# ZhangHH233/Retinal_OCT_Image_Segmentation_via_Deep_Learning

Measured on NVIDIA B200. Metric: bscans_per_sec_full_metric_suite, higher is better.
Workload: dtype u8

## Files before the change

retinal_oct_image_segmentation_via_deep_learning_b200/csrc/contour.cu:

```cuda
#include <cstdlib>
#include <cstring>
#include <numeric>
#include <type_traits>

#include <mutex>

#include "common.cuh"
#include "trace_core.h"

namespace octm {

struct TraceParams {
    const uint8_t* yt;
    const uint8_t* yp;
    long long n_items;
    int H, W, K, max_pts;
    const uint32_t* first_pos;
    uint32_t* verts;
    uint32_t* n_pts;
    uint32_t* flags;
    const int* bnd_t;
    const int* bnd_p;
    bool only_todo;
    const uint32_t* todo_count;
// ... 1133 lines not shown
                else break;
            }
            digit = static_cast<uint32_t>(lane * 8 + d);
            knew = k - run;
        }
        const int src = __ffs(__ballot_sync(0xffffffffu, mine)) - 1;
        digit = __shfl_sync(0xffffffffu, digit, src);
        k = __shfl_sync(0xffffffffu, knew, src);
        prefix |= digit << shift;
        maskbits |= 255u << shift;
        __syncwarp();
    }
    return prefix;
}

__global__ void __launch_bounds__(128) distance_select_kernel(const SelectParams prm) {
    __shared__ uint32_t s_hist[4][256];
    const int lane = threadIdx.x & 31, warp = threadIdx.x >> 5;
    const int cap = prm.max_pts;
    if (prm.todo_count != nullptr && *prm.todo_count == 0) return;
    for (long long unit = static_cast<long long>(blockIdx.x) * 4 + warp; unit < prm.n_units;
         unit += static_cast<long long>(gridDim.x) * 4) {
        const long long pair = unit >> 1;
        const int dir = static_cast<int>(unit & 1);
        if (prm.max_sq[unit] != kNeedsSelect) continue;
        const int nq = static_cast<int>(min(prm.n_pts[pair * 2 + 1 - dir], static_cast<uint32_t>(cap)));
        const uint32_t* dq = prm.d2 + unit * static_cast<long long>(cap);
        uint32_t vmax = 0;
        double dsum = 0.0;
        {
            double ds[4] = {0.0, 0.0, 0.0, 0.0};
            int j = lane;
            for (; j + 96 < nq; j += 128) {
                uint32_t v[4];
#pragma unroll
                for (int u = 0; u < 4; ++u) v[u] = dq[j + 32 * u];
#pragma unroll
                for (int u = 0; u < 4; ++u) {
                    vmax = max(vmax, v[u]);
                    ds[u] += sqrt(static_cast<double>(v[u]) / 4.0);
                }
            }
            double dt = 0.0;
            for (; j < nq; j += 32) {
                const uint32_t v = dq[j];
                vmax = max(vmax, v);
                dt += sqrt(static_cast<double>(v) / 4.0);
            }
            dsum = ((ds[0] + ds[1]) + (ds[2] + ds[3])) + dt;
        }
        vmax = __reduce_max_sync(0xffffffffu, vmax);
#pragma unroll
        for (int o = 16; o > 0; o >>= 1) dsum += __shfl_xor_sync(0xffffffffu, dsum, o);
        const double pos = __dmul_rn(static_cast<double>(nq - 1), 0.95);
        const uint32_t lo = static_cast<uint32_t>(floor(pos));
        const uint32_t v_lo = warp_select(dq, nq, lo, vmax, s_hist[warp], lane);
        uint32_t cnt_le = 0, next_gt = 0xffffffffu;
#pragma unroll 4
        for (int j = lane; j < nq; j += 32) {
            const uint32_t v = dq[j];
            cnt_le += v <= v_lo ? 1u : 0u;
            if (v > v_lo) next_gt = min(next_gt, v);
        }
        cnt_le = __reduce_add_sync(0xffffffffu, cnt_le);
        next_gt = __reduce_min_sync(0xffffffffu, next_gt);
        const uint32_t v_hi = (lo + 1 >= static_cast<uint32_t>(nq) || cnt_le >= lo + 2) ? v_lo : next_gt;
        if (lane == 0) {
            prm.max_sq[unit] = vmax;
            prm.p95_sq[unit * 2 + 0] = v_lo;
            prm.p95_sq[unit * 2 + 1] = v_hi;
            prm.sum_dist[unit] = dsum;
        }
    }
}


constexpr int kLdWarps = 4;
constexpr int kLdPad = 32;
constexpr int kLdRing = 512;
constexpr int kLdShort = 64;
#ifndef OCTM_LD_MINB
#define OCTM_LD_MINB 8
#endif

struct LayeredDistParams {
    const uint32_t* first_pos;
    const int* bnd_t;
    const int* bnd_p;
    const uint32_t* unsorted;
    long long n_pairs;
    int H, W, K, max_pts;
    int tab;
    uint32_t* verts;
    uint32_t* n_pts;
    uint32_t* max_sq;
    uint32_t* p95_sq;
    double* sum_dist;
    uint32_t* todo_count;
    uint32_t* search_count;
    int vals_cap;
};

__device__ __forceinline__ int max3i(int a, int b, int c) { return max(max(a, b), c); }
__device__ __forceinline__ int min3i(int a, int b, int c) { return min(min(a, b), c); }

__device__ __forceinline__ void layered_nearest2p(const short* lo0, const short* hi0, const short* lo1, const short* hi1, int qy0,
                                                  int qx0, int qy1, int qx1, int ncol, int& best0, int& best1) {
    const short* l0 = lo0 + qx0;
    const short* h0 = hi0 + qx0;
    const short* l1 = lo1 + qx1;
    const short* h1 = hi1 + qx1;
    const int dy0 = max3i(l0[0] - qy0, qy0 - h0[0], 0), dy1 = max3i(l1[0] - qy1, qy1 - h1[0], 0);
    best0 = dy0 * dy0;
    best1 = dy1 * dy1;
    int d = 1;
    while (d * d < max(best0, best1) && d < kLdPad) {
        const int d2 = d * d, e2 = (d + 1) * (d + 1);
        {
            const int a0 = max3i(l0[-d] - qy0, qy0 - h0[-d], 1), a1 = max3i(l0[d] - qy0, qy0 - h0[d], 1);
            const int b0 = max3i(l0[-d - 1] - qy0, qy0 - h0[-d - 1], 0), b1 = max3i(l0[d + 1] - qy0, qy0 - h0[d + 1], 0);
            best0 = min3i(best0, a0 * a0 + d2, a1 * a1 + d2);
            best0 = min3i(best0, b0 * b0 + e2, b1 * b1 + e2);
        }
        {
            const int a0 = max3i(l1[-d] - qy1, qy1 - h1[-d], 1), a1 = max3i(l1[d] - qy1, qy1 - h1[d], 1);
            const int b0 = max3i(l1[-d - 1] - qy1, qy1 - h1[-d - 1], 0), b1 = max3i(l1[d + 1] - qy1, qy1 - h1[d + 1], 0);
            best1 = min3i(best1, a0 * a0 + d2, a1 * a1 + d2);
            best1 = min3i(best1, b0 * b0 + e2, b1 * b1 + e2);
        }
        d += 2;
    }
    for (int e = d; e * e < best0; ++e) {
        const int cl = max(qx0 - e, -1), cr = min(qx0 + e, ncol), par = e & 1;
        const int a0 = max3i(lo0[cl] - qy0, qy0 - hi0[cl], par), a1 = max3i(lo0[cr] - qy0, qy0 - hi0[cr], par);
        best0 = min3i(best0, a0 * a0 + e * e, a1 * a1 + e * e);
    }
    for (int e = d; e * e < best1; ++e) {
        const int cl = max(qx1 - e, -1), cr = min(qx1 + e, ncol), par = e & 1;
        const int a0 = max3i(lo1[cl] - qy1, qy1 - hi1[cl], par), a1 = max3i(lo1[cr] - qy1, qy1 - hi1[cr], par);
        best1 = min3i(best1, a0 * a0 + e * e, a1 * a1 + e * e);
    }
}
__device__ __forceinline__ void layered_nearest2(const short* lo, const short* hi, int qy0, int qx0, int qy1, int qx1,
                                                 int ncol, int& best0, int& best1) {
    layered_nearest2p(lo, hi, lo, hi, qy0, qx0, qy1, qx1, ncol, best0, best1);
}

__device__ __forceinline__ void list_nearest2(const int2* pts, int n, int qy0, int qx0, int qy1, int qx1, int& best0, int& best1) {
    best0 = best1 = 0x7fffffff;
#pragma unroll 2
    for (int i = 0; i < n; ++i) {
        const int2 v = pts[i];
        const int dy0 = v.x - qy0, dx0 = v.y - qx0, dy1 = v.x - qy1, dx1 = v.y - qx1;
        best0 = min(best0, dy0 * dy0 + dx0 * dx0);
        best1 = min(best1, dy1 * dy1 + dx1 * dx1);
    }
}

struct LdSide {
    const short* lo;
    const short* hi;
    const int2* pts;
    const int* best;
    int n;
};

template <bool SRC_TABLE>
__device__ __forceinline__ void ld_list_minima(const int2* qpts, int nq, const LdSide& src, int ncol, int tid, int* best) {
    for (int q = 0; q < nq; ++q) {
        const int2 v = qpts[q];
        int b = 0x7fffffff;
        if (SRC_TABLE) {
            for (int c = tid; c < ncol; c += kLdWarps * 32) {
                const int dx = c - v.y;
                const int dy = max3i(src.lo[c] - v.x, v.x - src.hi[c], dx & 1);
                b = min(b, dy * dy + dx * dx);
            }
        } else {
            for (int i = tid; i < src.n; i += kLdWarps * 32) {
                const int dy = src.pts[i].x - v.x, dx = src.pts[i].y - v.y;
                b = min(b, dy * dy + dx * dx);
            }
        }
        b = __reduce_min_sync(0xffffffffu, b);
        if ((tid & 31) == 0) atomicMin(&best[q], b);
    }
}

template <bool SRC_TABLE>
__device__ __forceinline__ void ld_nearest2(const LdSide& src, int qy0, int qx0, int qy1, int qx1, int ncol, int& b0, int& b1) {
    if (SRC_TABLE) layered_nearest2(src.lo, src.hi, qy0, qx0, qy1, qx1, ncol, b0, b1);
    else list_nearest2(src.pts, src.n, qy0, qx0, qy1, qx1, b0, b1);
}

struct FineCounter {
    uint32_t* bins;
    uint32_t run_max = 0;
    bool run_bad = false, overflow = false;
    __device__ __forceinline__ void add(int best, bool valid, int lane) { count_minima(best, valid, lane, bins, run_max, run_bad); }
};
struct WideCounter {
    uint32_t* bins;
    int mode;
    int shift;
    uint32_t target;
    uint32_t run_max = 0, next_min = 0xffffffffu;
    double sum = 0.0;
    bool run_bad = false, overflow = false;
    uint32_t* vals = nullptr;
    uint32_t* vals_n = nullptr;
    __device__ __forceinline__ void add(int best, bool valid, int lane) {
        if (mode == 0) {
            count_minima(best, valid, lane, bins, run_max, run_bad);
            return;
        }
        if (mode == 1 && vals != nullptr) {
            const uint32_t m = __ballot_sync(0xffffffffu, valid);
            uint32_t base = 0;
            if (lane == 0 && m) base = atomicAdd(vals_n, static_cast<uint32_t>(__popc(m)));
            base = __shfl_sync(0xffffffffu, base, 0);
            if (valid) vals[base + __popc(m & lanemask_lt())] = static_cast<uint32_t>(best);
        }
        const uint32_t v = static_cast<uint32_t>(best), key = v >> shift;
        if (valid) run_max = max(run_max, v);
        const bool in = valid && (mode == 1 || key == target);
        const uint32_t idx = mode == 1 ? key : (v & ((1u << shift) - 1u)) >> 1;
        const uint32_t peers = __match_any_sync(0xffffffffu, in ? idx : static_cast<uint32_t>(kCountBins) + lane);
        if (in && lane == __ffs(peers) - 1) atomicAdd(&bins[idx >> 1], static_cast<uint32_t>(__popc(peers)) << ((idx & 1u) * 16));
// ... 69 lines not shown
        ld_nearest2<SRC_TABLE>(src, static_cast<int>(q0 >> 16), static_cast<int>(q0 & 0xffffu), static_cast<int>(q1 >> 16),
                               static_cast<int>(q1 & 0xffffu), ncol, b0, b1);
        ctr.add(b0, v0, lane);
        ctr.add(b1, v1, lane);
    }
}

__device__ __forceinline__ void ld_list_stats(const int* best, int n, int lane, uint32_t* max_sq, uint32_t* p95_sq, double* sum_dist) {
    const bool v0 = lane < n, v1 = lane + 32 < n;
    const uint32_t a = v0 ? static_cast<uint32_t>(best[lane]) : 0u, b = v1 ? static_cast<uint32_t>(best[lane + 32]) : 0u;
    uint32_t ra = 0, rb = 0;
    for (int i = 0; i < n; ++i) {
        const uint32_t w = static_cast<uint32_t>(best[i]);
        ra += (w < a || (w == a && i < lane)) ? 1u : 0u;
        rb += (w < b || (w == b && i < lane + 32)) ? 1u : 0u;
    }
    const double pos = __dmul_rn(static_cast<double>(n - 1), 0.95);
    const uint32_t lo = static_cast<uint32_t>(floor(pos)), hi = lo + 1 < static_cast<uint32_t>(n) ? lo + 1 : lo;
    uint32_t v_lo = 0, v_hi = 0;
    uint32_t m = __ballot_sync(0xffffffffu, v0 && ra == lo);
    if (m) v_lo = __shfl_sync(0xffffffffu, a, __ffs(m) - 1);
    m = __ballot_sync(0xffffffffu, v1 && rb == lo);
    if (m) v_lo = __shfl_sync(0xffffffffu, b, __ffs(m) - 1);
    m = __ballot_sync(0xffffffffu, v0 && ra == hi);
    if (m) v_hi = __shfl_sync(0xffffffffu, a, __ffs(m) - 1);
    m = __ballot_sync(0xffffffffu, v1 && rb == hi);
    if (m) v_hi = __shfl_sync(0xffffffffu, b, __ffs(m) - 1);
    const uint32_t vmax = __reduce_max_sync(0xffffffffu, max(a, b));
    double ds = __dadd_rn(v0 ? sqrt(static_cast<double>(a) / 4.0) : 0.0, v1 ? sqrt(static_cast<double>(b) / 4.0) : 0.0);
#pragma unroll
    for (int o = 16; o > 0; o >>= 1) ds = __dadd_rn(ds, __shfl_xor_sync(0xffffffffu, ds, o));
    if (lane == 0) {
        *max_sq = vmax;
        p95_sq[0] = v_lo;
        p95_sq[1] = v_hi;
        *sum_dist = ds;
    }
}

__device__ __forceinline__ void ld_table_vs_list(const short* qlo, const short* qhi, const int2* pts, int n, int W, int nq, int tid,
                                                 uint32_t* vals, uint32_t* s_nvals, uint32_t* s_scr , double* s_dscr ,
                                                 uint32_t* s_hist , uint32_t* s_bc , uint32_t* max_sq, uint32_t* p95_sq,
                                                 double* sum_dist) {
    uint32_t vmax = 0;
    double dsum = 0.0;
    auto emit = [&](int qy, int qx) {
        int best = 0x7fffffff;
        for (int i = 0; i < n; ++i) {
            const int2 v = pts[i];
            const int dy = v.x - qy, dx = v.y - qx;
            best = min(best, dy * dy + dx * dx);
        }
        vals[atomicAdd(s_nvals, 1u)] = static_cast<uint32_t>(best);
        vmax = max(vmax, static_cast<uint32_t>(best));
        dsum = __dadd_rn(dsum, sqrt(static_cast<double>(best) / 4.0));
    };
    for (int x = tid; x < W; x += kLdWarps * 32) {
        emit(qlo[2 * x], 2 * x);
        if (x + 1 < W)
            for (int y = qlo[2 * x + 1], yh = qhi[2 * x + 1]; y <= yh; y += 2) emit(y, 2 * x + 1);
    }
    vmax = block_reduce_max<kLdWarps * 32>(vmax, s_scr);
    dsum = block_reduce_add<kLdWarps * 32>(dsum, s_dscr);
    const double pos = __dmul_rn(static_cast<double>(nq - 1), 0.95);
    const uint32_t lo = static_cast<uint32_t>(floor(pos));
    const uint32_t v_lo = block_select<kLdWarps * 32>(vals, nq, lo, vmax, s_hist, s_bc);
    uint32_t cnt_le = 0, next_gt = 0xffffffffu;
    for (int j = tid; j < nq; j += kLdWarps * 32) {
        const uint32_t v = vals[j];
        cnt_le += v <= v_lo ? 1u : 0u;
        if (v > v_lo) next_gt = min(next_gt, v);
    }
    cnt_le = block_reduce_add<kLdWarps * 32>(cnt_le, s_scr);
    next_gt = block_reduce_min<kLdWarps * 32>(next_gt, s_scr);
    const uint32_t v_hi = (lo + 1 >= static_cast<uint32_t>(nq) || cnt_le >= lo + 2) ? v_lo : next_gt;
    if (tid == 0) {
        *max_sq = vmax;
        p95_sq[0] = v_lo;
        p95_sq[1] = v_hi;
        *sum_dist = dsum;
    }
}

__device__ __forceinline__ void ld_both_tt(const short* tabs, int tab, int W, int ncol, int warp, int lane, uint32_t* ring,
                                           uint32_t* bins2, uint32_t* s_vmax, uint32_t* s_bad) {
    uint32_t rm0 = 0, rm1 = 0, head = 0, tail = 0;
    bool bad0 = false, bad1 = false, overflow = false;
    const int nblk = (W + 63) >> 6;
    auto count = [&](int bestd, bool valid, uint32_t dirq) {
        const uint32_t dv = static_cast<uint32_t>(bestd), h = dv >> 1;
        const bool ok = valid && (dv & 1u) == 0 && h < static_cast<uint32_t>(kCountBins);
        const uint32_t peers = __match_any_sync(0xffffffffu, ok ? (h | (dirq << 16)) : 0x100000u + lane);
        if (ok && lane == __ffs(peers) - 1)
            atomicAdd(&bins2[dirq * (kCountBins / 2) + (h >> 1)], static_cast<uint32_t>(__popc(peers)) << ((h & 1u) * 16));
        if (valid) {
            if (dirq) rm1 = max(rm1, dv); else rm0 = max(rm0, dv);
            if (!ok) { if (dirq) bad1 = true; else bad0 = true; }
        }
    };
    auto ring_round = [&](uint32_t left) {
        const bool v0 = static_cast<uint32_t>(lane) < left, v1 = static_cast<uint32_t>(lane) + 32u < left;
        const uint32_t idle = static_cast<uint32_t>(static_cast<unsigned short>(tabs[kLdPad])) << 16;
        const uint32_t q0 = v0 ? ring[(head + lane) & (kLdRing - 1)] : idle, q1 = v1 ? ring[(head + 32 + lane) & (kLdRing - 1)] : idle;
        head += left < 64u ? left : 64u;
        const uint32_t d0 = q0 >> 31, d1 = q1 >> 31;
        const short* lo0 = tabs + kLdPad + d0 * (2 * tab);
        const short* lo1 = tabs + kLdPad + d1 * (2 * tab);
        int b0, b1;
        layered_nearest2p(lo0, lo0 + tab, lo1, lo1 + tab, static_cast<int>((q0 >> 16) & 0x7fffu), static_cast<int>(q0 & 0xffffu),
                          static_cast<int>((q1 >> 16) & 0x7fffu), static_cast<int>(q1 & 0xffffu), ncol, b0, b1);
        count(b0, v0, d0);
        count(b1, v1, d1);
    };
#pragma unroll 1
    for (int dir = 0; dir < 2 && !overflow; ++dir) {
        const short* slo = tabs + kLdPad + dir * (2 * tab);
        const short* shi = slo + tab;
        const short* qlo = tabs + kLdPad + (1 - dir) * (2 * tab);
        const short* qhi = qlo + tab;
        const uint32_t tag = static_cast<uint32_t>(dir) << 31;
        const int idle_y = slo[0];
        for (int blk = warp; blk < nblk; blk += kLdWarps) {
            const int xa = blk * 64 + lane, xb = xa + 32;
            const bool va = xa < W, vb = xb < W;
            int ba, bb;
            layered_nearest2(slo, shi, va ? qlo[2 * xa] : idle_y, va ? 2 * xa : 0, vb ? qlo[2 * xb] : idle_y, vb ? 2 * xb : 0, ncol, ba, bb);
            count(ba, va, static_cast<uint32_t>(dir));
            count(bb, vb, static_cast<uint32_t>(dir));
            const bool ra = xa + 1 < W, rb = xb + 1 < W;
            const int la = ra ? qlo[2 * xa + 1] : 32767, ha = ra ? qhi[2 * xa + 1] : -32768;
            const int lb = rb ? qlo[2 * xb + 1] : 32767, hb = rb ? qhi[2 * xb + 1] : -32768;
            const uint32_t lena = ha >= la ? static_cast<uint32_t>((ha - la) >> 1) + 1u : 0u;
            const uint32_t lenb = hb >= lb ? static_cast<uint32_t>((hb - lb) >> 1) + 1u : 0u;
            const uint32_t len = lena + lenb;
            uint32_t incl = len;
#pragma unroll
            for (int o = 1; o < 32; o <<= 1) {
                const uint32_t up = __shfl_up_sync(0xffffffffu, incl, o);
                if (lane >= o) incl += up;
            }
            const uint32_t total = __shfl_sync(0xffffffffu, incl, 31);
            if (total > static_cast<uint32_t>(kLdRing - 64)) { overflow = true; break; }
            uint32_t at = tail + incl - len;
            for (uint32_t t = 0; t < lena; ++t, ++at)
                ring[at & (kLdRing - 1)] = tag | (static_cast<uint32_t>(la + 2 * static_cast<int>(t)) << 16) | static_cast<uint32_t>(2 * xa + 1);
            for (uint32_t t = 0; t < lenb; ++t, ++at)
                ring[at & (kLdRing - 1)] = tag | (static_cast<uint32_t>(lb + 2 * static_cast<int>(t)) << 16) | static_cast<uint32_t>(2 * xb + 1);
            tail += total;
            __syncwarp();
            while (tail - head >= 64u) ring_round(64u);
            __syncwarp();
        }
    }
    if (!overflow && tail != head) ring_round(tail - head);
    const uint32_t w0 = __reduce_max_sync(0xffffffffu, rm0), w1 = __reduce_max_sync(0xffffffffu, rm1);
    const bool b0 = __any_sync(0xffffffffu, bad0), b1 = __any_sync(0xffffffffu, bad1), ov = __any_sync(0xffffffffu, overflow);
    if (lane == 0) {
        atomicMax(&s_vmax[0], w0);
        atomicMax(&s_vmax[1], w1);
        if (b0 || b1 || ov) atomicOr(s_bad, (b0 ? 1u : 0u) | (b1 ? 2u : 0u) | (ov ? 4u : 0u));
    }
}

__device__ __forceinline__ void ld_emit(const short* lo, const short* hi, int ncol, int lane, uint32_t* out, uint32_t cap) {
    uint32_t base = 0;
    for (int c0 = 0; c0 < ncol; c0 += 32) {
        const int c = c0 + lane;
        const int l = c < ncol ? lo[c] : 32767, h = c < ncol ? hi[c] : -32768;
        const uint32_t len = h >= l ? static_cast<uint32_t>((h - l) >> 1) + 1u : 0u;
        uint32_t incl = len;
#pragma unroll
        for (int o = 1; o < 32; o <<= 1) {
            const uint32_t up = __shfl_up_sync(0xffffffffu, incl, o);
            if (lane >= o) incl += up;
        }
        uint32_t at = base + incl - len;
        for (uint32_t t = 0; t < len; ++t, ++at)
            if (at < cap) out[at] = (static_cast<uint32_t>(l + 2 * static_cast<int>(t)) << 16) | static_cast<uint32_t>(c);
        base += __shfl_sync(0xffffffffu, incl, 31);
    }
}

template <int PASS>
__global__ void __launch_bounds__(kLdWarps * 32, PASS != 2 ? OCTM_LD_MINB : 8) layered_distance_kernel(const LayeredDistParams prm) {
    extern __shared__ __align__(16) uint8_t dsm[];
    __shared__ uint32_t s_vmax[2], s_bad, s_ok[2], s_minkey[2], s_cnt[2], s_seed[2];
    __shared__ int2 s_list[2][kLdShort];
    __shared__ int s_lbest[2][kLdShort];
    __shared__ double s_dsum[kLdWarps];
    __shared__ double s_dsum8[8];
    __shared__ uint32_t s_next, s_tgt[3], s_amax, s_nvals;
    constexpr bool P1 = PASS == 1 || PASS == 3;
    const int tid = threadIdx.x, lane = tid & 31, warp = tid >> 5;
    const int W = prm.W, K = prm.K, tab = prm.tab, ncol = 2 * W - 1;
    if (PASS == 2 && *prm.todo_count == 0) return;
    short* const tabs = reinterpret_cast<short*>(dsm);
    uint32_t* const bins2 = reinterpret_cast<uint32_t*>(dsm + static_cast<size_t>(tab) * 8);
    uint32_t* const ring = bins2 + kCountBins + warp * kLdRing;
    for (int i = tid; i < kCountBins; i += kLdWarps * 32) bins2[i] = 0;
    for (int i = tid; i < 2 * tab; i += kLdWarps * 32) {
        const int m = i >= tab ? 1 : 0, j = i - m * tab;
        if (j < kLdPad || j >= kLdPad + ncol) {
            tabs[(2 * m) * tab + j] = 32767;
            tabs[(2 * m + 1) * tab + j] = -32768;
        }
    }

    for (long long pair0 = blockIdx.x; pair0 < prm.n_pairs; pair0 += gridDim.x) {
      bool own_next = false;
      for (int rep = 0; rep < 2; ++rep) {
        if (rep == 1 && !own_next) break;
        const long long pair = pair0 + rep;
        if (PASS == 2 && prm.max_sq[pair * 2] != kNeedsSearch) continue;
        __syncthreads();
        const long long item = pair / K;
        const int cls = static_cast<int>(pair - item * K);
        if (P1 && rep == 0) {
            const uint32_t ft = lane < K ? prm.first_pos[(item * 2 + 0) * K + lane] : OCTM_NO_SEED;
            const uint32_t fq = lane < K ? prm.first_pos[(item * 2 + 1) * K + lane] : OCTM_NO_SEED;
            const int c00t = __ffs(__ballot_sync(0xffffffffu, ft == 0u)) - 1, c00p = __ffs(__ballot_sync(0xffffffffu, fq == 0u)) - 1;
            if (c00t >= 0 && c00t == c00p && (PASS != 3 || (prm.unsorted[item] & 3u) == 0u)) {
                if (cls == c00t + 1) break;
                own_next = cls == c00t && cls + 1 < K;
            }
        }
        if (tid < 2) { s_vmax[tid] = 0; s_ok[tid] = 1; s_minkey[tid] = 0xffffffffu; s_cnt[tid] = 0; }
        if (tid == 2) s_bad = 0;
        const uint32_t unsorted = P1 ? prm.unsorted[item] : 0u;
        uint32_t n0 = 0, n1 = 0;
        if (PASS == 2 || (PASS == 3 && (unsorted & 1u))) n0 = prm.n_pts[pair * 2];
        if (PASS == 2 || (PASS == 3 && (unsorted & 2u))) n1 = prm.n_pts[pair * 2 + 1];
        const bool row0 = PASS == 3 && (unsorted & 1u) && n0 != kTraceTodo && (n0 & kRowBit);
        const bool row1 = PASS == 3 && (unsorted & 2u) && n1 != kTraceTodo && (n1 & kRowBit);
        __syncthreads();
        {
            const int m = warp >> 1;
            const uint32_t nm = m ? n1 : n0;
            const bool rowside = PASS == 3 && ((unsorted >> m) & 1u) && nm != kTraceTodo && (nm & kRowBit);
            const bool want = P1 || (nm != kTraceTodo && (nm & kLayeredBit));
            const uint32_t* fp = prm.first_pos + (item * 2 + m) * K;
            const uint32_t myfp = lane < K ? fp[lane] : OCTM_NO_SEED;
            const int c00 = __ffs(__ballot_sync(0xffffffffu, myfp == 0u)) - 1;
            const bool inv = cls == c00;
            const uint32_t others = __reduce_min_sync(0xffffffffu, lane == c00 ? OCTM_NO_SEED : myfp);
            const uint32_t seed = inv ? others : __shfl_sync(0xffffffffu, myfp, cls);
            if (lane == 0 && (warp & 1) == 0) s_seed[m] = seed;
            const int brow = inv ? cls : cls - 1;
            if (want && seed != OCTM_NO_SEED && (!((unsorted >> m) & 1u) || rowside) && brow >= 0 && brow < K - 1) {
                const int* rows = (m ? prm.bnd_p : prm.bnd_t) + item * (K - 1) * static_cast<long long>(W);
                const int* hrow = rows + brow * static_cast<long long>(W);
                if ((PASS == 2 && (nm & kRowBit)) || rowside)
                    hrow = reinterpret_cast<const int*>(prm.verts + (pair * 2 + m) * static_cast<long long>(prm.max_pts));
                const int* orow = inv ? (cls > 0 ? rows + (cls - 1) * static_cast<long long>(W) : nullptr)
                                      : (cls < K - 1 ? rows + cls * static_cast<long long>(W) : nullptr);
                if (PASS == 2 || rowside) orow = nullptr;
                uint32_t* lo32 = reinterpret_cast<uint32_t*>(tabs + (2 * m) * tab + kLdPad);
                uint32_t* hi32 = lo32 + (tab >> 1);
                bool ok = true;
                uint32_t minkey = 0xffffffffu, steps = 0;
                const int H = prm.H;
                const bool vec4 = (W & 3) == 0 && ((reinterpret_cast<uintptr_t>(hrow) | reinterpret_cast<uintptr_t>(orow)) & 15) == 0;
                for (int x0 = (warp & 1) * 128; vec4 && x0 < W; x0 += 256) {
                    const int x = x0 + 4 * lane;
                    const int xc = min(x, W - 4);
                    const int4 hv = *reinterpret_cast<const int4*>(hrow + xc);
                    const int4 ov = orow != nullptr ? *reinterpret_cast<const int4*>(orow + xc) : (inv ? make_int4(0, 0, 0, 0) : make_int4(H, H, H, H));
                    int hl = __shfl_up_sync(0xffffffffu, hv.w, 1), hn = __shfl_down_sync(0xffffffffu, hv.x, 1);
                    if (lane == 0) hl = hrow[max(xc - 1, 0)];
                    if (lane == 31) hn = hrow[min(xc + 4, W - 1)];
                    if (x + 4 >= W) hn = hv.w;
                    if (x < W) {
                        const int hh[6] = {hl, hv.x, hv.y, hv.z, hv.w, hn};
                        const int oo[4] = {ov.x, ov.y, ov.z, ov.w};
                        uint32_t wl[4], wh[4];
#pragma unroll
                        for (int i = 0; i < 4; ++i) {
                            const int h = hh[i + 1], hp = hh[i], hx = hh[i + 2];
                            if (P1) {
                                const int lo_w = min(hp, min(h, hx)), hi_w = max(hp, max(h, hx));
                                ok = ok && h >= 1 && h <= H - 1 && (inv ? oo[i] <= lo_w - 1 : oo[i] >= hi_w + 1);
                                minkey = min(minkey, static_cast<uint32_t>(h) * static_cast<uint32_t>(W) + static_cast<uint32_t>(x + i));
// ... 517 lines not shown
        if (smem > static_cast<size_t>(octm::max_optin_smem()))
            return octm::fail(OCTM_ERR_UNSUPPORTED, "tile %d needs %zu B of shared memory", tile, smem);
        if (cudaFuncSetAttribute(octm::distance_search_kernel, cudaFuncAttributeMaxDynamicSharedMemorySize,
                                 static_cast<int>(smem)) != cudaSuccess)
            return octm::fail(OCTM_ERR_LAUNCH, "cudaFuncSetAttribute(distance_search_kernel) failed");
        octm::SearchParams sp{verts, n_pts, n_pairs * 2, max_pts, tile, d2, max_sq, p95_sq, sum_dist, keep_d2 != 0, only_marked, todo_count};
        long long grid = n_pairs * 2;
        const long long cap = static_cast<long long>(octm::sm_count()) * 32;
        if (grid > cap) grid = cap;
        OCTM_TIMED("distance_search_kernel", st) octm::distance_search_kernel<<<static_cast<unsigned>(grid), octm::kSearchThreads, smem, st>>>(sp);
        if (int e = octm::check_launch("distance_search_kernel")) return e;
        return run_select();
    }
    const size_t smem = dist_smem(max_pts);
    if (smem > static_cast<size_t>(octm::max_optin_smem()) - 4096)
        return octm::fail(OCTM_ERR_UNSUPPORTED, "max_pts %d needs %zu B of shared memory in this mode", max_pts, smem);
    octm::DistParams p{verts, n_pts, n_pairs, max_pts, max_sq, p95_sq, sum_dist, d2};
    long long grid = n_pairs;
    const long long cap = static_cast<long long>(octm::sm_count()) * 16;
    if (grid > cap) grid = cap;
    auto kern = mode == 2 ? octm::distance_kernel<false> : octm::distance_kernel<true>;
    if (cudaFuncSetAttribute(kern, cudaFuncAttributeMaxDynamicSharedMemorySize, octm::max_optin_smem() - 4096) != cudaSuccess)
        return octm::fail(OCTM_ERR_LAUNCH, "cudaFuncSetAttribute(distance_kernel) failed");
    OCTM_TIMED("distance_kernel", st) kern<<<static_cast<unsigned>(grid), octm::kDistThreads, smem, st>>>(p);
    return octm::check_launch("distance_kernel");
}

extern "C" int octm_contour2d_distance(const uint32_t* verts, const uint32_t* n_pts, int64_t n_items, int num_classes,
                                       int max_pts, int H, int W, uint32_t* max_sq, uint32_t* p95_sq, double* sum_dist,
                                       uint32_t* d2, int keep_d2, void* stream) {
    return run_distance(verts, n_pts, n_items, num_classes, max_pts, H, W, max_sq, p95_sq, sum_dist, d2, keep_d2, false, nullptr, stream);
}

namespace octm {
__global__ void walk_report_kernel(const uint32_t* walk_count, uint32_t contours, uint32_t* out) {
    out[1] = contours;
    out[0] = *walk_count;
}
struct WalkReport {
    uint32_t* host = nullptr;
    uint32_t* dev = nullptr;
};
static WalkReport g_walk_report[64];
static std::mutex g_walk_mu;
static WalkReport* walk_report() {
    int dev = -1;
    if (cudaGetDevice(&dev) != cudaSuccess || dev < 0 || dev >= 64) { cudaGetLastError(); return nullptr; }
    std::lock_guard<std::mutex> lk(g_walk_mu);
    WalkReport& r = g_walk_report[dev];
    if (r.host == nullptr) {
        void* h = nullptr;
        void* d = nullptr;
        if (cudaHostAlloc(&h, 2 * sizeof(uint32_t), cudaHostAllocMapped) != cudaSuccess || cudaHostGetDevicePointer(&d, h, 0) != cudaSuccess) {
            cudaGetLastError();
            return nullptr;
        }
        r.host = static_cast<uint32_t*>(h);
        r.dev = static_cast<uint32_t*>(d);
        r.host[0] = r.host[1] = 0;
    }
    return &r;
}
}

extern "C" int octm_contour2d_metrics_u8(const uint8_t* y_true, const uint8_t* y_pred, int64_t n_items, int H, int W,
                                         int num_classes, const uint32_t* first_pos, const int32_t* bnd_true,
                                         const int32_t* bnd_pred, const uint32_t* unsorted, int max_pts, uint32_t* n_pts,
                                         uint32_t* flags, uint32_t* max_sq, uint32_t* p95_sq, double* sum_dist,
                                         void* workspace, size_t workspace_bytes, void* stream) {
    if (int e = check_shape(n_items, H, W, num_classes, max_pts)) return e;
    if (n_items == 0) return OCTM_OK;
    if (!y_true || !y_pred || !first_pos || !n_pts || !flags || !max_sq || !p95_sq || !sum_dist)
        return octm::fail(OCTM_ERR_INVALID, "null pointer");
    if ((bnd_true == nullptr) != (bnd_pred == nullptr)) return octm::fail(OCTM_ERR_INVALID, "bnd_true/bnd_pred: both or neither");
    const size_t verts_b = (static_cast<size_t>(n_items) * num_classes * 2 * max_pts * sizeof(uint32_t) + 255) & ~static_cast<size_t>(255);
    if (workspace == nullptr || workspace_bytes < 2 * verts_b + 256)
        return octm::fail(OCTM_ERR_WORKSPACE, "workspace too small: need %zu B", 2 * verts_b + 256);
    uint32_t* verts = static_cast<uint32_t*>(workspace);
    uint32_t* d2 = reinterpret_cast<uint32_t*>(static_cast<uint8_t*>(workspace) + verts_b);
    uint32_t* todo = reinterpret_cast<uint32_t*>(static_cast<uint8_t*>(workspace) + 2 * verts_b);
    cudaStream_t s = static_cast<cudaStream_t>(stream);
    static const bool env_fused = [] { const char* e = getenv("OCTM_LAYERED_FUSED"); return !(e && e[0] == '0'); }();
    const int tab = (2 * W - 1 + 2 * octm::kLdPad + 7) & ~7;
    const size_t smem = static_cast<size_t>(tab) * 8 + octm::kCountBins * 4 + octm::kLdWarps * octm::kLdRing * 4;
    const bool fused = env_fused && unsorted != nullptr && layered_ok(y_true, y_pred, bnd_true, bnd_pred, H, W, num_classes) &&
                       H <= 4095 && max_pts <= 0xffff && smem <= static_cast<size_t>(octm::max_optin_smem());
    if (!fused) {
        if (int e = octm_contour2d_trace_u8(y_true, y_pred, n_items, H, W, num_classes, first_pos, bnd_true, bnd_pred, max_pts,
                                            verts, n_pts, flags, stream))
            return e;
        return run_distance(verts, n_pts, n_items, num_classes, max_pts, H, W, max_sq, p95_sq, sum_dist, d2, 0, false, nullptr, stream);
    }
    if (cudaMemsetAsync(flags, 0, sizeof(uint32_t) * n_items * num_classes, s) != cudaSuccess ||
        cudaMemsetAsync(todo, 0, 3 * sizeof(uint32_t), s) != cudaSuccess)
        return octm::fail(OCTM_ERR_LAUNCH, "memset(flags) failed");
    uint32_t* search = todo + 1;
    const long long n_pairs = n_items * num_classes;
    octm::LayeredDistParams lp{first_pos, bnd_true, bnd_pred, unsorted, n_pairs, H, W, num_classes, max_pts, tab, verts,
                               n_pts, max_sq, p95_sq, sum_dist, todo, search, 0};
    auto launch_fused = [&](int pass) -> int {
        auto kern = pass == 1 ? octm::layered_distance_kernel<1> : (pass == 3 ? octm::layered_distance_kernel<3> : octm::layered_distance_kernel<2>);
        size_t smem_pass = smem;
        lp.vals_cap = 0;
        if (pass == 2 && max_pts <= 4096) {
            smem_pass += static_cast<size_t>(max_pts) * 4;
            lp.vals_cap = max_pts;
        }
        const size_t smem = smem_pass;
        if (cudaFuncSetAttribute(kern, cudaFuncAttributeMaxDynamicSharedMemorySize, static_cast<int>(smem)) != cudaSuccess)
            return octm::fail(OCTM_ERR_LAUNCH, "cudaFuncSetAttribute(layered_distance_kernel) failed");
        int fit = 0;
        if (cudaOccupancyMaxActiveBlocksPerMultiprocessor(&fit, kern, octm::kLdWarps * 32, smem) != cudaSuccess || fit < 1) {
            cudaGetLastError();
            fit = 1;
        }
        static const int env_ctas = [] { const char* e = getenv("OCTM_LD_CTAS"); return e ? atoi(e) : 0; }();
        if (env_ctas > 0 && env_ctas < fit) fit = env_ctas;
        long long grid = n_pairs;
        const long long cap = static_cast<long long>(octm::sm_count()) * fit;
        if (grid > cap) grid = cap;
        while (grid > 1 && std::gcd(grid, static_cast<long long>(num_classes)) != 1) --grid;
        OCTM_TIMED(pass == 1 ? "layered_distance_kernel" : (pass == 3 ? "layered_distance_kernel_rows" : "layered_distance_kernel_pass2"), s)
            kern<<<static_cast<unsigned>(grid), octm::kLdWarps * 32, smem, s>>>(lp);
        return octm::check_launch("layered_distance_kernel");
    };
    octm::TraceParams p{y_true, y_pred, n_items, H, W, num_classes, max_pts, first_pos, verts, n_pts, flags,
                        bnd_true, bnd_pred, true, todo, d2, todo + 2, 0, unsorted, 0};
    octm::WalkReport* wr = octm::stream_mostly_rejected() ? octm::walk_report() : nullptr;
    const bool few_walks = wr != nullptr && (octm_label_pass_seed_policy(-1) == 2 ||
                                             static_cast<unsigned long long>(*static_cast<volatile uint32_t*>(wr->host)) * 4ull <=
                                                 *static_cast<volatile uint32_t*>(wr->host + 1));
    if (wr != nullptr && few_walks) {
        p.take = 1;
        p.todo_count = nullptr;
        if (int e = launch_layered_trace<false>(p, s)) return e;
        p.todo_count = todo;
        if (int e = launch_fused(3)) return e;
        p.take = 2;
    } else {
        if (int e = launch_fused(1)) return e;
    }
    if (int e = launch_layered_trace<false>(p, s)) return e;
    p.take = 0;
    if (wr != nullptr) {
        OCTM_TIMED("walk_report_kernel", s) octm::walk_report_kernel<<<1, 1, 0, s>>>(
            todo + 2, static_cast<uint32_t>(std::min<long long>(n_items * num_classes * 2, 0xffffffffll)), wr->dev);
        if (int e = octm::check_launch("walk_report_kernel")) return e;
    }
    if (int e = launch_walk(p, s)) return e;
    if (int e = launch_fused(2)) return e;
    return run_distance(verts, n_pts, n_items, num_classes, max_pts, H, W, max_sq, p95_sq, sum_dist, d2, 0, true, search, stream);
}

extern "C" size_t octm_contour2d_workspace_bytes(int64_t n_items, int H, int W, int num_classes, int max_pts) {
    (void)H; (void)W;
    if (n_items <= 0 || num_classes < 1 || max_pts < 1) return 0;
    const size_t verts = static_cast<size_t>(n_items) * num_classes * 2 * max_pts * sizeof(uint32_t);
    const size_t first = static_cast<size_t>(n_items) * 2 * num_classes * sizeof(uint32_t);
    return 2 * ((verts + 255) & ~static_cast<size_t>(255)) + ((first + 255) & ~static_cast<size_t>(255));
}

extern "C" int octm_contour2d_u8(const uint8_t* y_true, const uint8_t* y_pred, int64_t n_items, int H, int W,
                                 int num_classes, const uint32_t* first_pos, int max_pts, uint32_t* n_pts,
                                 uint32_t* flags, uint32_t* max_sq, uint32_t* p95_sq, double* sum_dist, void* workspace,
                                 size_t workspace_bytes, void* stream) {
    if (int e = check_shape(n_items, H, W, num_classes, max_pts)) return e;
    if (n_items == 0) return OCTM_OK;
    if (workspace == nullptr || workspace_bytes < octm_contour2d_workspace_bytes(n_items, H, W, num_classes, max_pts))
        return octm::fail(OCTM_ERR_WORKSPACE, "workspace too small: need %zu B",
                          octm_contour2d_workspace_bytes(n_items, H, W, num_classes, max_pts));
    uint32_t* verts = static_cast<uint32_t*>(workspace);
    const size_t verts_b = (static_cast<size_t>(n_items) * num_classes * 2 * max_pts * sizeof(uint32_t) + 255) & ~static_cast<size_t>(255);
    uint32_t* d2_ws = reinterpret_cast<uint32_t*>(static_cast<uint8_t*>(workspace) + verts_b);
    uint32_t* fp_ws = reinterpret_cast<uint32_t*>(static_cast<uint8_t*>(workspace) + 2 * verts_b);
    if (first_pos == nullptr) {
        const long long grid = n_items < 148 * 8 ? n_items : 148 * 8;
        cudaStream_t s = static_cast<cudaStream_t>(stream);
        OCTM_TIMED("first_pos_kernel", s) octm::first_pos_kernel<<<static_cast<unsigned>(grid), 256, 0, s>>>(y_true, n_items, static_cast<long long>(H) * W,
                                                                         num_classes, fp_ws, 2 * num_classes);
        if (int e = octm::check_launch("first_pos_kernel")) return e;
        OCTM_TIMED("first_pos_kernel", s) octm::first_pos_kernel<<<static_cast<unsigned>(grid), 256, 0, s>>>(y_pred, n_items, static_cast<long long>(H) * W,
                                                                         num_classes, fp_ws + num_classes, 2 * num_classes);
        if (int e = octm::check_launch("first_pos_kernel")) return e;
        first_pos = fp_ws;
    }
// ... 6 lines not shown
```

Before: 3.407 million.

## Restructure layered nearest search into per-lane slot scheduler with work queue

```diff
diff --git a/retinal_oct_image_segmentation_via_deep_learning_b200/csrc/contour.cu b/retinal_oct_image_segmentation_via_deep_learning_b200/csrc/contour.cu
--- a/retinal_oct_image_segmentation_via_deep_learning_b200/csrc/contour.cu
+++ b/retinal_oct_image_segmentation_via_deep_learning_b200/csrc/contour.cu
@@ -1239,6 +1239,14 @@
 #ifndef OCTM_LD_MINB
 #define OCTM_LD_MINB 8
 #endif
+#ifndef OCTM_LD_SLOTS
+#define OCTM_LD_SLOTS 2
+#endif
+constexpr int kLdSlots = OCTM_LD_SLOTS;
+constexpr int kLdQueue = 128;
+constexpr int kLdCbuf = 128;
+static_assert(32 * (kLdSlots + 1) <= kLdQueue && 32 * (kLdSlots + 1) <= kLdCbuf, "PASS 1 queue sizes");
+__host__ __device__ constexpr int ld_warp_words(int pass) { return pass == 2 ? kLdRing : kLdQueue + kLdCbuf; }
 
 struct LayeredDistParams {
     const uint32_t* first_pos;
@@ -1261,12 +1269,21 @@
 __device__ __forceinline__ int max3i(int a, int b, int c) { return max(max(a, b), c); }
 __device__ __forceinline__ int min3i(int a, int b, int c) { return min(min(a, b), c); }
 
-__device__ __forceinline__ void layered_nearest2p(const short* lo0, const short* hi0, const short* lo1, const short* hi1, int qy0,
-                                                  int qx0, int qy1, int qx1, int ncol, int& best0, int& best1) {
-    const short* l0 = lo0 + qx0;
-    const short* h0 = hi0 + qx0;
-    const short* l1 = lo1 + qx1;
-    const short* h1 = hi1 + qx1;
+__device__ __forceinline__ int layered_far(const short* lo, const short* hi, int qy, int qx, int ncol, int d, int best) {
+    for (int e = d; e * e < best; ++e) {
+        const int cl = max(qx - e, -1), cr = min(qx + e, ncol), par = e & 1;
+        const int a0 = max3i(lo[cl] - qy, qy - hi[cl], par), a1 = max3i(lo[cr] - qy, qy - hi[cr], par);
+        best = min3i(best, a0 * a0 + e * e, a1 * a1 + e * e);
+    }
+    return best;
+}
+
+__device__ __forceinline__ void layered_nearest2(const short* lo, const short* hi, int qy0, int qx0, int qy1, int qx1,
+                                                 int ncol, int& best0, int& best1) {
+    const short* l0 = lo + qx0;
+    const short* h0 = hi + qx0;
+    const short* l1 = lo + qx1;
+    const short* h1 = hi + qx1;
     const int dy0 = max3i(l0[0] - qy0, qy0 - h0[0], 0), dy1 = max3i(l1[0] - qy1, qy1 - h1[0], 0);
     best0 = dy0 * dy0;
     best1 = dy1 * dy1;
@@ -1287,20 +1304,8 @@
         }
         d += 2;
     }
-    for (int e = d; e * e < best0; ++e) {
-        const int cl = max(qx0 - e, -1), cr = min(qx0 + e, ncol), par = e & 1;
-        const int a0 = max3i(lo0[cl] - qy0, qy0 - hi0[cl], par), a1 = max3i(lo0[cr] - qy0, qy0 - hi0[cr], par);
-        best0 = min3i(best0, a0 * a0 + e * e, a1 * a1 + e * e);
-    }
-    for (int e = d; e * e < best1; ++e) {
-        const int cl = max(qx1 - e, -1), cr = min(qx1 + e, ncol), par = e & 1;
-        const int a0 = max3i(lo1[cl] - qy1, qy1 - hi1[cl], par), a1 = max3i(lo1[cr] - qy1, qy1 - hi1[cr], par);
-        best1 = min3i(best1, a0 * a0 + e * e, a1 * a1 + e * e);
-    }
-}
-__device__ __forceinline__ void layered_nearest2(const short* lo, const short* hi, int qy0, int qx0, int qy1, int qx1,
-                                                 int ncol, int& best0, int& best1) {
-    layered_nearest2p(lo, hi, lo, hi, qy0, qx0, qy1, qx1, ncol, best0, best1);
+    best0 = layered_far(lo, hi, qy0, qx0, ncol, d, best0);
+    best1 = layered_far(lo, hi, qy1, qx1, ncol, d, best1);
 }
 
 __device__ __forceinline__ void list_nearest2(const int2* pts, int n, int qy0, int qx0, int qy1, int qx1, int& best0, int& best1) {
@@ -1536,15 +1541,16 @@
     }
 }
 
-__device__ __forceinline__ void ld_both_tt(const short* tabs, int tab, int W, int ncol, int warp, int lane, uint32_t* ring,
+__device__ __forceinline__ void ld_both_tt(const short* tabs, int tab, int W, int ncol, int warp, int lane, uint32_t* queue,
                                            uint32_t* bins2, uint32_t* s_vmax, uint32_t* s_bad) {
-    uint32_t rm0 = 0, rm1 = 0, head = 0, tail = 0;
+    constexpr uint32_t kAll = 0xffffffffu, kNoSeg = 0x80000000u;
+    uint32_t* const cbuf = queue + kLdQueue;
+    uint32_t rm0 = 0, rm1 = 0;
     bool bad0 = false, bad1 = false, overflow = false;
-    const int nblk = (W + 63) >> 6;
-    auto count = [&](int bestd, bool valid, uint32_t dirq) {
-        const uint32_t dv = static_cast<uint32_t>(bestd), h = dv >> 1;
+    auto count = [&](uint32_t v, bool valid) {
+        const uint32_t dirq = v >> 31, dv = v & 0x7fffffffu, h = dv >> 1;
         const bool ok = valid && (dv & 1u) == 0 && h < static_cast<uint32_t>(kCountBins);
-        const uint32_t peers = __match_any_sync(0xffffffffu, ok ? (h | (dirq << 16)) : 0x100000u + lane);
+        const uint32_t peers = __match_any_sync(kAll, ok ? (h | (dirq << 16)) : 0x100000u + lane);
         if (ok && lane == __ffs(peers) - 1)
             atomicAdd(&bins2[dirq * (kCountBins / 2) + (h >> 1)], static_cast<uint32_t>(__popc(peers)) << ((h & 1u) * 16));
         if (valid) {
@@ -1552,63 +1558,140 @@
             if (!ok) { if (dirq) bad1 = true; else bad0 = true; }
         }
     };
-    auto ring_round = [&](uint32_t left) {
-        const bool v0 = static_cast<uint32_t>(lane) < left, v1 = static_cast<uint32_t>(lane) + 32u < left;
-        const uint32_t idle = static_cast<uint32_t>(static_cast<unsigned short>(tabs[kLdPad])) << 16;
-        const uint32_t q0 = v0 ? ring[(head + lane) & (kLdRing - 1)] : idle, q1 = v1 ? ring[(head + 32 + lane) & (kLdRing - 1)] : idle;
-        head += left < 64u ? left : 64u;
-        const uint32_t d0 = q0 >> 31, d1 = q1 >> 31;
-        const short* lo0 = tabs + kLdPad + d0 * (2 * tab);
-        const short* lo1 = tabs + kLdPad + d1 * (2 * tab);
-        int b0, b1;
-        layered_nearest2p(lo0, lo0 + tab, lo1, lo1 + tab, static_cast<int>((q0 >> 16) & 0x7fffu), static_cast<int>(q0 & 0xffffu),
-                          static_cast<int>((q1 >> 16) & 0x7fffu), static_cast<int>(q1 & 0xffffu), ncol, b0, b1);
-        count(b0, v0, d0);
-        count(b1, v1, d1);
+    const int nblk = (W + 63) >> 6;
+    int g = warp, x0 = 0, qoff = 0, cseg = -1;
+    uint32_t tag = 0, total = 0, pos = 0, cstart = 0, sa = kNoSeg, sb = kNoSeg;
+    uint32_t qhead = 0, qtail = 0, chead = 0, ctail = 0;
+    auto load_block = [&]() {
+        const int dir = g >= nblk ? 1 : 0;
+        x0 = (g - dir * nblk) * 64;
+        qoff = kLdPad + (1 - dir) * (2 * tab);
+        tag = static_cast<uint32_t>(dir) << 31;
+        auto seg_len = [&](int x) -> uint32_t {
+            if (x >= W) return 0u;
+            if (x + 1 >= W) return 1u;
+            const int l = tabs[qoff + 2 * x + 1], h = tabs[qoff + tab + 2 * x + 1];
+            return 1u + (h >= l ? min(static_cast<uint32_t>((h - l) >> 1) + 1u, static_cast<uint32_t>(kLdRing - 63)) : 0u);
+        };
+        const uint32_t la = seg_len(x0 + lane), lb = seg_len(x0 + lane + 32);
+        uint32_t incl = la | (lb << 16);
+#pragma unroll
+        for (int o = 1; o < 32; o <<= 1) {
+            const uint32_t up = __shfl_up_sync(kAll, incl, o);
+            if (lane >= o) incl += up;
+        }
+        const uint32_t tot = __shfl_sync(kAll, incl, 31), ta = tot & 0xffffu;
+        total = ta + (tot >> 16);
+        sa = la ? (incl & 0xffffu) - la : kNoSeg;
+        sb = lb ? ta + (incl >> 16) - lb : kNoSeg;
+        pos = 0;
+        cseg = -1;
+        cstart = 0;
+        overflow = total - static_cast<uint32_t>(min(W - x0, 64)) > static_cast<uint32_t>(kLdRing - 64);
     };
+    auto produce = [&]() {
+        const uint32_t ra = sa - pos, rb = sb - pos;
+        const uint32_t m = __reduce_or_sync(kAll, (ra < 32u ? 1u << ra : 0u) | (rb < 32u ? 1u << rb : 0u));
+        const uint32_t le = m & (kAll >> (31 - lane));
+        const int seg = cseg + __popc(le);
+        const int t = le ? lane - (31 - __clz(le)) : static_cast<int>(pos - cstart) + lane;
+        const uint32_t n = min(total - pos, 32u);
+        if (static_cast<uint32_t>(lane) < n) {
+            const int c = 2 * (x0 + seg) + (t > 0 ? 1 : 0);
+            const int y = tabs[qoff + c] + 2 * max(t - 1, 0);
+            queue[(qtail + lane) & (kLdQueue - 1)] = tag | (static_cast<uint32_t>(y) << 16) | static_cast<uint32_t>(c);
+        }
+        qtail += n;
+        if (m) {
+            cseg += __popc(m);
+            cstart = pos + 31 - __clz(m);
+        }
+        pos += 32;
+    };
+    bool more = g < 2 * nblk;
+    if (more) {
+        load_block();
+        more = !overflow;
+    }
+    int qy[kLdSlots], off[kLdSlots], best[kLdSlots], d[kLdSlots];
+    bool act[kLdSlots];
+#pragma unroll
+    for (int s = 0; s < kLdSlots; ++s) {
+        qy[s] = 0;
+        off[s] = kLdPad;
+        best[s] = 0;
+        d[s] = 0;
+        act[s] = false;
+    }
 #pragma unroll 1
-    for (int dir = 0; dir < 2 && !overflow; ++dir) {
-        const short* slo = tabs + kLdPad + dir * (2 * tab);
-        const short* shi = slo + tab;
-        const short* qlo = tabs + kLdPad + (1 - dir) * (2 * tab);
-        const short* qhi = qlo + tab;
-        const uint32_t tag = static_cast<uint32_t>(dir) << 31;
-        const int idle_y = slo[0];
-        for (int blk = warp; blk < nblk; blk += kLdWarps) {
-            const int xa = blk * 64 + lane, xb = xa + 32;
-            const bool va = xa < W, vb = xb < W;
-            int ba, bb;
-            layered_nearest2(slo, shi, va ? qlo[2 * xa] : idle_y, va ? 2 * xa : 0, vb ? qlo[2 * xb] : idle_y, vb ? 2 * xb : 0, ncol, ba, bb);
-            count(ba, va, static_cast<uint32_t>(dir));
-            count(bb, vb, static_cast<uint32_t>(dir));
-            const bool ra = xa + 1 < W, rb = xb + 1 < W;
-            const int la = ra ? qlo[2 * xa + 1] : 32767, ha = ra ? qhi[2 * xa + 1] : -32768;
-            const int lb = rb ? qlo[2 * xb + 1] : 32767, hb = rb ? qhi[2 * xb + 1] : -32768;
-            const uint32_t lena = ha >= la ? static_cast<uint32_t>((ha - la) >> 1) + 1u : 0u;
-            const uint32_t lenb = hb >= lb ? static_cast<uint32_t>((hb - lb) >> 1) + 1u : 0u;
-            const uint32_t len = lena + lenb;
-            uint32_t incl = len;
-#pragma unroll
-            for (int o = 1; o < 32; o <<= 1) {
-                const uint32_t up = __shfl_up_sync(0xffffffffu, incl, o);
-                if (lane >= o) incl += up;
-            }
-            const uint32_t total = __shfl_sync(0xffffffffu, incl, 31);
-            if (total > static_cast<uint32_t>(kLdRing - 64)) { overflow = true; break; }
-            uint32_t at = tail + incl - len;
-            for (uint32_t t = 0; t < lena; ++t, ++at)
-                ring[at & (kLdRing - 1)] = tag | (static_cast<uint32_t>(la + 2 * static_cast<int>(t)) << 16) | static_cast<uint32_t>(2 * xa + 1);
-            for (uint32_t t = 0; t < lenb; ++t, ++at)
-                ring[at & (kLdRing - 1)] = tag | (static_cast<uint32_t>(lb + 2 * static_cast<int>(t)) << 16) | static_cast<uint32_t>(2 * xb + 1);
-            tail += total;
-            __syncwarp();
-            while (tail - head >= 64u) ring_round(64u);
-            __syncwarp();
-        }
-    }
-    if (!overflow && tail != head) ring_round(tail - head);
-    const uint32_t w0 = __reduce_max_sync(0xffffffffu, rm0), w1 = __reduce_max_sync(0xffffffffu, rm1);
-    const bool b0 = __any_sync(0xffffffffu, bad0), b1 = __any_sync(0xffffffffu, bad1), ov = __any_sync(0xffffffffu, overflow);
+    for (;;) {
+        __syncwarp();
+        while (more && qtail - qhead < 32u * kLdSlots) {
+            produce();
+            if (pos >= total) {
+                g += kLdWarps;
+                more = g < 2 * nblk;
+                if (more) {
+                    load_block();
+                    more = !overflow;
+                }
+            }
+        }
+        if (overflow) break;
+        __syncwarp();
+        const uint32_t avail = qtail - qhead;
+        uint32_t taken = 0;
+        bool busy = false;
+#pragma unroll
+        for (int s = 0; s < kLdSlots; ++s) {
+            const uint32_t need = __ballot_sync(kAll, !act[s]);
+            const uint32_t r = taken + __popc(need & lanemask_lt());
+            if (!act[s] && r < avail) {
+                const uint32_t e = queue[(qhead + r) & (kLdQueue - 1)];
+                qy[s] = static_cast<int>((e >> 16) & 0x7fffu);
+                off[s] = kLdPad + static_cast<int>(e >> 31) * (2 * tab) + static_cast<int>(e & 0xffffu);
+                best[s] = 0x7fffffff;
+                d[s] = 0;
+                act[s] = true;
+            }
+            taken += __popc(need);
+            busy = busy || act[s];
+        }
+        qhead += min(taken, avail);
+        if (!__any_sync(kAll, busy)) break;
+#pragma unroll
+        for (int s = 0; s < kLdSlots; ++s) {
+            const short* l = tabs + off[s];
+            const short* h = l + tab;
+            const int y = qy[s], a = d[s], b = a + 1, a2 = a * a, b2 = b * b;
+            const int a0 = max3i(l[-a] - y, y - h[-a], 0), a1 = max3i(l[a] - y, y - h[a], 0);
+            const int b0 = max3i(l[-b] - y, y - h[-b], 1), b1 = max3i(l[b] - y, y - h[b], 1);
+            best[s] = min3i(best[s], a0 * a0 + a2, a1 * a1 + a2);
+            best[s] = min3i(best[s], b0 * b0 + b2, b1 * b1 + b2);
+        }
+#pragma unroll
+        for (int s = 0; s < kLdSlots; ++s) {
+            const int nd = d[s] + 2, dir = off[s] >= 2 * tab ? 1 : 0;
+            const bool fin = act[s] && !(nd * nd < best[s] && nd < kLdPad);
+            if (fin && nd * nd < best[s]) {
+                const short* lo = tabs + kLdPad + dir * (2 * tab);
+                best[s] = layered_far(lo, lo + tab, qy[s], off[s] - kLdPad - dir * (2 * tab), ncol, nd, best[s]);
+            }
+            const uint32_t fm = __ballot_sync(kAll, fin);
+            if (fin) cbuf[(ctail + __popc(fm & lanemask_lt())) & (kLdCbuf - 1)] = static_cast<uint32_t>(best[s]) | (static_cast<uint32_t>(dir) << 31);
+            ctail += __popc(fm);
+            act[s] = act[s] && !fin;
+            d[s] = act[s] ? nd : 0;
+        }
+        __syncwarp();
+        for (; ctail - chead >= 32u; chead += 32u) count(cbuf[(chead + lane) & (kLdCbuf - 1)], true);
+    }
+    if (!overflow && ctail != chead) {
+        const bool v = static_cast<uint32_t>(lane) < ctail - chead;
+        count(v ? cbuf[(chead + lane) & (kLdCbuf - 1)] : 0u, v);
+    }
+    const uint32_t w0 = __reduce_max_sync(kAll, rm0), w1 = __reduce_max_sync(kAll, rm1);
+    const bool b0 = __any_sync(kAll, bad0), b1 = __any_sync(kAll, bad1), ov = __any_sync(kAll, overflow);
     if (lane == 0) {
         atomicMax(&s_vmax[0], w0);
         atomicMax(&s_vmax[1], w1);
@@ -1650,7 +1733,7 @@
     if (PASS == 2 && *prm.todo_count == 0) return;
     short* const tabs = reinterpret_cast<short*>(dsm);
     uint32_t* const bins2 = reinterpret_cast<uint32_t*>(dsm + static_cast<size_t>(tab) * 8);
-    uint32_t* const ring = bins2 + kCountBins + warp * kLdRing;
+    uint32_t* const ring = bins2 + kCountBins + warp * ld_warp_words(PASS);
     for (int i = tid; i < kCountBins; i += kLdWarps * 32) bins2[i] = 0;
     for (int i = tid; i < 2 * tab; i += kLdWarps * 32) {
         const int m = i >= tab ? 1 : 0, j = i - m * tab;
@@ -2334,7 +2417,10 @@
     cudaStream_t s = static_cast<cudaStream_t>(stream);
     static const bool env_fused = [] { const char* e = getenv("OCTM_LAYERED_FUSED"); return !(e && e[0] == '0'); }();
     const int tab = (2 * W - 1 + 2 * octm::kLdPad + 7) & ~7;
-    const size_t smem = static_cast<size_t>(tab) * 8 + octm::kCountBins * 4 + octm::kLdWarps * octm::kLdRing * 4;
+    auto ld_smem = [&](int pass) {
+        return static_cast<size_t>(tab) * 8 + octm::kCountBins * 4 + static_cast<size_t>(octm::kLdWarps) * octm::ld_warp_words(pass) * 4;
+    };
+    const size_t smem = std::max(ld_smem(1), ld_smem(2));
     const bool fused = env_fused && unsorted != nullptr && layered_ok(y_true, y_pred, bnd_true, bnd_pred, H, W, num_classes) &&
                        H <= 4095 && max_pts <= 0xffff && smem <= static_cast<size_t>(octm::max_optin_smem());
     if (!fused) {
@@ -2352,7 +2438,7 @@
                                n_pts, max_sq, p95_sq, sum_dist, todo, search, 0};
     auto launch_fused = [&](int pass) -> int {
         auto kern = pass == 1 ? octm::layered_distance_kernel<1> : (pass == 3 ? octm::layered_distance_kernel<3> : octm::layered_distance_kernel<2>);
-        size_t smem_pass = smem;
+        size_t smem_pass = ld_smem(pass);
         lp.vals_cap = 0;
         if (pass == 2 && max_pts <= 4096) {
             smem_pass += static_cast<size_t>(max_pts) * 4;
```

After: 2.725 million (median of 6 runs). -20.0%, worse.
